# google/bayesnf

Hardware: AMD Instinct MI355X
Metric: train-steps/sec x ensemble_size (member-steps/s, whole job) (higher is better)
Workload: dtype bf16; 1 GPU; C2 chickenpox-like MAP: N=10232 rows, D=3, F=57, width=512, depth=2, NORMAL, full batch, lr=0.005; members_per_gpu=64, ensemble_size=64, parallelism=ensemble-shard x1 (no data-path collective)

## Files before the change

bayesnf_amd/csrc/bnf_api.hip:

```cpp
#include <hip/hip_runtime.h>
#include <cstring>
#include <rocprim/device/device_radix_sort.hpp>
#include <rocprim/device/device_segmented_radix_sort.hpp>

#include <dlfcn.h>

#include <atomic>
#include <cmath>
#include <cstdarg>
#include <cstdio>
#include <cstdlib>
#include <cstring>
#include <string>
#include <vector>

#include "../../include/bnf.h"
#include "bnf_gemm.h"
#include "bnf_kernels.h"
#include "bnf_panel.h"
#include "bnf_gemm8.h"

using namespace bnf;

static thread_local char g_err[512] = "";
// ... 74 lines not shown
  void* H0 = nullptr; void* H0t = nullptr;
  const float* ext_eps = nullptr;
  const uint32_t* vi_keys = nullptr; int64_t vi_key_rows = 0, vi_key_t0 = 0;
  const uint32_t* vi_draw_keys = nullptr; int64_t vi_draw_rows = 0;
  const int32_t* row_tab = nullptr; int64_t row_tab_epochs = 0, row_tab_e0 = 0;
  const uint32_t* row_keys = nullptr; int64_t row_keys_epochs = 0, row_keys_e0 = 0; int32_t row_key_rounds = 0;
  uint32_t* perm_bits[2] = {nullptr, nullptr}; int32_t* perm_val[2] = {nullptr, nullptr};
  unsigned* perm_seg = nullptr; void* perm_tmp = nullptr; size_t perm_tmp_bytes = 0;
  bool perm_ready = false;
  size_t owned_bytes = 0;
  int32_t* perm = nullptr; int64_t perm_epoch = -1;
  int32_t* leaf_off = nullptr; uint8_t* leaf_id = nullptr; int32_t n_leaves = 0;
  bool adam_clear_all = false;
  bool h0l = false;
  bool fold0 = false;
  void* A[BNF_MAX_LAYERS]; void* H[BNF_MAX_LAYERS]; void* Ht[BNF_MAX_LAYERS];
  void* dZ[BNF_MAX_LAYERS]; void* dZt[BNF_MAX_LAYERS];
  void* Kn[BNF_MAX_LAYERS]; void* Kt[BNF_MAX_LAYERS];
  int64_t pack_batch[BNF_MAX_LAYERS];
  float* dH0 = nullptr; float* out = nullptr; float* ybat = nullptr; float* loss_raw = nullptr;
  float* vacc = nullptr; float* dv = nullptr;
  bool vi_sample_pack = true, vi_keep_z = false;
  bool panel = false;
  void* Wf[BNF_MAX_LAYERS]; void* Wb[BNF_MAX_LAYERS];
  void* park[BNF_MAX_LAYERS];
    unsigned long long* prof_buf = nullptr;
  double prof_gap[16] = {0, 0, 0, 0, 0, 0, 0, 0, 0, 0, 0, 0, 0, 0, 0, 0};
  double prof_blocks = 0;
  int prof_threads = 0;
  bool recompute_a0 = false;
  bool fuse_last = false;
  int num_cus = 256;
  int tn_ring = 1;
  int skinny = 1;
  int big_tiles = 1;
  float* scal = nullptr;
  StepState* step_state = nullptr;
  hipGraphExec_t graph_exec = nullptr;
  int64_t graph_cols = 0;
  float* graph_losses = nullptr;
  int graph_mode = 0;
  float* qscratch = nullptr;
  float* dbg_a = nullptr; float* dbg_b = nullptr;
  uint8_t* is_matrix = nullptr;
  size_t ws_bytes = 0;
  int ablate = 0;
// ... 45 lines not shown
    h->dZ[l] = fo ? nullptr : take((size_t)Ev * Bp * W * es);
    h->dZt[l] = nullptr;
    const int64_t npad = (l == 0) ? Fp : W;
    h->pack_batch[l] = npad * W;
    h->Kn[l] = h->panel ? nullptr : take((size_t)Ev * npad * W * es);
    h->Kt[l] = h->panel ? nullptr : take((size_t)Ev * npad * W * es);
  }
  for (int l = 0; l < h->L; ++l) {
    const int64_t npad = (l == 0) ? Fp : W;
    h->Wf[l] = h->panel ? take((size_t)Ev * npad * W * es) : nullptr;
    h->Wb[l] = h->panel ? take((size_t)Ev * npad * W * es) : nullptr;
    h->park[l] = (h->panel && !fo && l >= 1 && l < h->L - 1) ? take((size_t)Ev * Bp * W * es) : nullptr;
    h->Wf8[l] = (h->c8 && l >= 1) ? (uint8_t*)take((size_t)Ev * W * W) : nullptr;
    h->Wb8[l] = (h->c8 && l >= 1) ? (uint8_t*)take((size_t)Ev * W * W) : nullptr;
  }
  h->dH0 = fo ? nullptr : (float*)take((size_t)Ev * Fp * Bp * 4);
  h->out = (float*)take((size_t)Ev * Bp * 4);
  h->vacc = (float*)take((size_t)Ev * Bp * 4);
  h->dv = fo ? nullptr : (float*)take((size_t)Ev * Bp * 4);
  h->ybat = fo ? nullptr : (float*)take((size_t)Ev * Bp * 4);
  h->loss_raw = (float*)take((size_t)Ev * 4);
  h->qscratch = (float*)take((size_t)(4 * 1024 + 16) * 4);
  h->scal = (float*)take((size_t)Ev * kScalStride * 4);
  h->step_state = (StepState*)take(sizeof(StepState));
  h->dbg_a = (float*)take(256);
  h->is_matrix = (uint8_t*)take((size_t)P);
  h->fbmeta = h->fbmeta_h.empty() ? nullptr : (int32_t*)take(h->fbmeta_h.size() * 4);
  if (h->cfg.mode == BNF_MODE_VI) {
    h->leaf_off = (int32_t*)take(260 * 4);
    h->leaf_id = (uint8_t*)take((size_t)P);
  }
  return off;
}

struct LaunchScope {
  bnf_handle* h;
  int kid;
  hipEvent_t t0 = nullptr, t1 = nullptr;
  bool on;
  hipStream_t st;
  LaunchScope(bnf_handle* h_, int kid_, hipStream_t st_ = nullptr, bool use_st = false)
      : h(h_), kid(kid_), on(((h_->prof >> kid_) & 1u) != 0), st(use_st ? st_ : h_->stream) {
    if (!on) return;
    auto get = [&]() {
      if (h->pool_used == h->event_pool.size()) {
        hipEvent_t ev;
// ... 565 lines not shown
    jb.off_kernel[l] = h->nd.off_kernel[l];
    jb.n_in[l] = (l == 0) ? h->F : h->W;
    jb.n_pad[l] = (l == 0) ? h->Fp : h->W;
    jb.tile0[l] = tiles;
    tiles += (jb.n_pad[l] / 64) * (h->W / 64);
    jb.wf[l] = h->Wf[l]; jb.wb[l] = h->Wb[l]; jb.batch[l] = h->pack_batch[l];
  }
  jb.tile0[h->L] = tiles;
  jb.fold0 = h->fold0 ? 1 : 0; jb.F0n = h->F; jb.off_bias0 = h->nd.off_bias[0]; jb.off_ls0 = h->nd.off_ls[0];
  for (int l = 0; l < h->L; ++l) { jb.wf8[l] = h->Wf8[l]; jb.wb8[l] = h->Wb8[l]; }
  jb.batch8 = (int64_t)h->W * h->W;
  *n_tiles = tiles;
  return jb;
}
template <typename T>
static void run_pack_fragments(bnf_handle* h, const float* theta, int nmem) {
  LaunchScope ls(h, KID_PACK);
  int tiles = 0;
  const PackJobs jb = pack_jobs(h, &tiles);
  hipLaunchKernelGGL((k_pack_layers<T>), dim3((unsigned)tiles * (unsigned)nmem), dim3(256), 0, h->stream,
                     theta, (int64_t)h->Pf, jb, h->nd, h->scal);
}

template <int WN, int RT, bool H0L, bool DEEP, int CH, int FP, bool F0, bool C8 = false>
static void launch_panel_f(bnf_handle* h, const PanelArgs& pa) {
  constexpr int kLds = panel_lds_bytes(WN, RT, H0L, CH, FP);
  static_assert(kLds <= 160 * 1024, "LDS per workgroup");
  static std::atomic<uint64_t> attr_done{0};
  allow_lds(h, &k_panel_fwd_bwd<WN, RT, H0L, DEEP, CH, FP, F0, C8>, kLds, &attr_done);
  PanelArgs pa2 = pa;
  pa2.ablate = h->ablate;
  const unsigned blocks = (unsigned)(pa.members * pa.panels);
  {
    EpiArgs tmp{};
    phase_prof_begin(h, KID_PANEL, blocks, &tmp);
    pa2.prof = tmp.prof;
  }
  {
    LaunchScope ls(h, KID_PANEL);
    hipLaunchKernelGGL((k_panel_fwd_bwd<WN, RT, H0L, DEEP, CH, FP, F0, C8>), dim3(blocks), dim3(512), kLds, h->stream, pa2);
  }
  phase_prof_end(h, KID_PANEL, blocks, 512);
}
template <int WN, int RT, bool H0L, bool DEEP, int CH, int FP>
static void launch_panel_d(bnf_handle* h, const PanelArgs& pa) {
  if constexpr (H0L) {
    if (h->fold0) {
      if (pa.c8) {
        launch_panel_f<WN, RT, H0L, DEEP, CH, FP, true, true>(h, pa);
        return;
      }
      launch_panel_f<WN, RT, H0L, DEEP, CH, FP, true>(h, pa);
      return;
    }
  }
  launch_panel_f<WN, RT, H0L, DEEP, CH, FP, false>(h, pa);
}

template <int WN, int RT, bool H0L, int CH = 1, int FP = 64>
static void launch_panel(bnf_handle* h, const PanelArgs& pa) {
  if (pa.n_layers == 2) launch_panel_d<WN, RT, H0L, false, CH, FP>(h, pa);
  else launch_panel_d<WN, RT, H0L, true, CH, FP>(h, pa);
}

static void run_panel(bnf_handle* h, const float* theta, int nmem, const RowSrc& rs, float c,
// ... 214 lines not shown
  } else {
    run_pack<T>(h, thf, E);
    run_forward<T>(h, thf, E, rs, h->X, h->stab, h->y, h->B, true);
    run_backward<T>(h, thf, E, rs, h->B, c, sink);
  }
  fold_grad(h, E);
  AdamArgs a{};
  a.theta = h->params; a.m = h->state; a.v = h->state + (int64_t)E * h->P; a.grad = h->grad;
  a.stride = h->P; a.P = h->P; a.off_shape = h->nd.off_shape;
  const int64_t t = h->adam_t + 1;
  a.lr = h->cfg.learning_rate;
  a.bc1 = (float)(1.0 - std::pow(0.9, (double)t));
  a.bc2 = (float)(1.0 - std::pow(0.999, (double)t));
  a.prior_weight = h->cfg.prior_weight;
  a.loss = sink.loss; a.loss_stride = sink.stride; a.loss_scale = sink.scale;
  a.apply = apply ? 1 : 0; a.loss_raw = sink.raw; a.st = sink.st;
  a.keep_lo = a.keep_hi = 0;
  if (!h->pad && !h->adam_clear_all && h->ablate == 0)
    for (int l = 1; l < h->L; ++l)
      if (wgrad_splitk(h, E, l) == 1 && a.keep_hi == 0) {
        a.keep_lo = (h->nd.off_kernel[l] + 3) / 4 * 4;
        a.keep_hi = (h->nd.off_kernel[l] + h->W * h->W) / 4 * 4;
      }
  {
    LaunchScope ls(h, KID_ADAM);
    hipLaunchKernelGGL(k_adam_map, dim3(cdiv(cdiv(h->P, 4), 256 * BNF_ADAM_QUADS), (unsigned)E), dim3(256), 0, h->stream, a);
  }
  if (apply) h->adam_t = t;
  return BNF_OK;
}

static ViSegs vi_segments_all(const bnf_handle* h) {
  ViSegs sg{};
  sg.n = 1; sg.lo[0] = 0; sg.hi[0] = h->P;
  return sg;
}
static ViSegs vi_segments_between_kernels(const bnf_handle* h) {
  ViSegs sg{};
  int32_t at = 0;
  for (int l = 0; l < h->L; ++l) {
    sg.lo[sg.n] = at; sg.hi[sg.n] = h->nd.off_kernel[l]; ++sg.n;
    at = h->nd.off_kernel[l] + ((l == 0) ? h->F : h->W) * h->W;
  }
  sg.lo[sg.n] = at; sg.hi[sg.n] = h->P; ++sg.n;
  return sg;
}
static dim3 vi_sample_grid(const ViSegs& sg, int members) {
  int32_t longest = 1;
  for (int i = 0; i < sg.n; ++i) longest = std::max(longest, sg.hi[i] - sg.lo[i]);
// ... 234 lines not shown
    int want = cfg->pipeline;
    if (const char* pf = getenv("BNF_PIPELINE")) want = atoi(pf);
    if (want != 0 && want != 1 && want != 3) {
      delete h;
      return fail(BNF_ERR_INVALID, "pipeline %d (0 auto, 1 layers, 3 panel)", want);
    }
    const bool can_panel = !cfg->forward_only && h->bf16 && h->L >= 2 && (h->W == 256 || h->W == 512 || h->W == 1024) && h->Fp <= 128;
    if (want == 3 && !can_panel) {
      delete h;
      return fail(BNF_ERR_INVALID, "panel pipeline needs a bf16 training handle with depth >= 2, width 256/512/1024 and <= 128 features");
    }
    h->panel = can_panel && (want == 3 || want == 0);
    if (h->q8 && !h->panel && !cfg->forward_only) {
      delete h;
      return fail(BNF_ERR_INVALID, "dtype fp8 (fp8 operand storage for the weight gradients) needs the row-panel pipeline: "
                  "depth >= 2, width 256 / 512 / 1024 after padding to 64, <= 128 padded features");
    }
    if (h->panel) h->Bp = align_up(h->B, 256);
    h->c8 = h->q8 && h->panel && !(getenv("BNF_FP8_CONTRACT") && atoi(getenv("BNF_FP8_CONTRACT")) == 0);
    const bool fl_ok = h->bf16 ? fused_last_supported<bf16_t>(h->W) : fused_last_supported<float>(h->W);
    h->fuse_last = !cfg->forward_only && !h->panel && want == 0 && fl_ok;
    h->recompute_a0 = !cfg->forward_only && !h->panel && want == 0 && h->L >= 2 && h->Fp <= 128;
  }
  h->h0l = panel_h0l(h);
  h->fold0 = h->h0l && h->F + 2 <= h->Fp && !(getenv("BNF_PANEL_FOLD0") && atoi(getenv("BNF_PANEL_FOLD0")) == 0);
  h->c8 = h->c8 && h->fold0;
  if (h->h0l &&
      !(getenv("BNF_PANEL_FEATBWD") && atoi(getenv("BNF_PANEL_FEATBWD")) == 0)) {
    int in_group = -1;
    for (int g = 0; g < cfg->n_groups; ++g)
      if (cfg->group_kind[g] == BNF_GROUP_INPUT) in_group = g;
    if (in_group >= 0) {
      std::vector<int32_t>& m = h->fbmeta_h;
      const int Fp = h->Fp;
      m.assign(Fp * 4 + BNF_MAX_GROUPS, 0);
      auto put = [&](int col, int kind, int g, int d1, int d2, int partner, int ucol, float coef) {
        m[4 * col] = kind | (g << 8) | (d1 << 16) | (d2 << 24);
        m[4 * col + 1] = partner | (ucol << 8);
        memcpy(&m[4 * col + 2], &coef, 4);
      };
      for (int c = 0; c < Fp; ++c) put(c, kFbNone, 0xff, 0xff, 0xff, 0, 0, 0.f);
      const int cin = cfg->group_col0[in_group];
      for (int g = 0; g < cfg->n_groups; ++g) {
        const int c0 = cfg->group_col0[g], nc = cfg->group_ncols[g];
        m[4 * Fp + g] = cfg->group_scale_off[g];
        switch (cfg->group_kind[g]) {
// ... 809 lines not shown
```

bayesnf_amd/csrc/bnf_kernels.h:

```cpp
#pragma once

#include "bnf_device.h"
#include "../../include/bnf.h"

namespace bnf {

constexpr int kScalGroup = BNF_MAX_LAYERS + 2;
constexpr int kScalInput = kScalGroup + BNF_MAX_GROUPS;
constexpr int kScalGfac = kScalInput + BNF_MAX_INPUTS;
constexpr int kScalStride = kScalGfac + BNF_MAX_GROUPS;

__device__ __forceinline__ void sincos_rev(float x, float* s, float* c) {
  sincosf(6.28318530717958647692f * x, s, c);
}

struct NetDev {
  int32_t D, F, Fp, W, Wt, depth, P, n_groups, n_freqs, n_interact, obs;
  int32_t group_kind[BNF_MAX_GROUPS], group_arg[BNF_MAX_GROUPS], group_ncols[BNF_MAX_GROUPS],
      group_col0[BNF_MAX_GROUPS], group_scale_off[BNF_MAX_GROUPS];
  int32_t fdeg[BNF_MAX_INPUTS];
  float in_scale[BNF_MAX_INPUTS];
  int32_t interact[BNF_MAX_INTERACT][2];
  int32_t off_lns, off_shape, off_infl;
  int32_t off_bias[BNF_MAX_LAYERS + 1], off_kernel[BNF_MAX_LAYERS + 1], off_ls[BNF_MAX_LAYERS];
// ... 553 lines not shown
  }
  theta_pad[(int64_t)e * Pp + j] = v;
}
__global__ void k_fold_grad(float* __restrict__ grad_pad, int64_t Pp, const int32_t* __restrict__ fold_src,
                            float* __restrict__ grad, int64_t P) {
  const int e = blockIdx.y;
  const int64_t i = (int64_t)blockIdx.x * blockDim.x + threadIdx.x;
  if (i >= P) return;
  grad[(int64_t)e * P + i] = grad_pad[(int64_t)e * Pp + fold_src[i]];
}

struct AdamArgs {
  float* theta; float* m; float* v; float* grad;
  int64_t stride;
  int32_t P;
  int32_t off_shape;
  float lr, bc1, bc2;
  float prior_weight;
  float* loss; int64_t loss_stride; float loss_scale;
  int32_t apply;
  float* loss_raw;
  const StepState* st;
  int32_t keep_lo, keep_hi;
};

__global__ void k_step_advance(StepState* st) {
  if (threadIdx.x == 0 && blockIdx.x == 0) {
    const long long t = st->t + 1;
    st->t = t;
    st->col += 1;
    st->bc1 = (float)(1.0 - pow(0.9, (double)t));
    st->bc2 = (float)(1.0 - pow(0.999, (double)t));
  }
}

#ifndef BNF_ADAM_QUADS
#define BNF_ADAM_QUADS 4
#endif
__global__ __launch_bounds__(256) void k_adam_map(AdamArgs a) {
  __shared__ float red[4];
  const int e = blockIdx.y;
  const float bc1 = a.st ? a.st->bc1 : a.bc1, bc2 = a.st ? a.st->bc2 : a.bc2;
  float lp = 0.f;
#pragma unroll
  for (int qd = 0; qd < BNF_ADAM_QUADS; ++qd) {
  const int p0 = ((blockIdx.x * BNF_ADAM_QUADS + qd) * blockDim.x + threadIdx.x) * 4;
  if (p0 < a.P) {
    const int nv = min(4, a.P - p0);
    const int64_t i0 = (int64_t)e * a.stride + p0;
    float th[4], g[4], m[4], v[4];
    load4u(a.theta + i0, nv, th); load4u(a.grad + i0, nv, g);
    if (a.apply) { load4u(a.m + i0, nv, m); load4u(a.v + i0, nv, v); }
    const float ibc1 = 1.0f / bc1, ibc2 = 1.0f / bc2;
#pragma unroll
    for (int k = 0; k < 4; ++k) {
      if (a.prior_weight != 0.f && k < nv) {
        const float z = th[k] - ((p0 + k) == a.off_shape ? -1.5f : 0.f);
        const float az = fabsf(z);
        const float e = __builtin_amdgcn_exp2f(-1.44269504088896340736f * az);
        const float r = __builtin_amdgcn_rcpf(1.0f + e);
        g[k] += a.prior_weight * copysignf((1.0f - e) * r, z);
        lp += -az - 1.38629436111989061883f * __builtin_amdgcn_logf(1.0f + e);
      }
      if (a.apply) {
        m[k] = 0.9f * m[k] + 0.1f * g[k];
        v[k] = 0.999f * v[k] + 0.001f * g[k] * g[k];
        th[k] = th[k] - a.lr * (m[k] * ibc1) * __builtin_amdgcn_rcpf(__builtin_amdgcn_sqrtf(v[k] * ibc2) + 1e-8f);
        g[k] = 0.f;
      }
    }
    if (!(a.apply && p0 >= a.keep_lo && p0 < a.keep_hi)) store4u(a.grad + i0, nv, g);
    if (a.apply) {
      store4u(a.theta + i0, nv, th);
      store4u<true>(a.m + i0, nv, m);
      store4u<true>(a.v + i0, nv, v);
    }
  }
  }
  const float s = wave_sum(lp);
  if ((threadIdx.x & 63) == 0) red[threadIdx.x >> 6] = s;
  __syncthreads();
  if (threadIdx.x == 0 && a.prior_weight != 0.f) {
    const float t = -(a.prior_weight) * (red[0] + red[1] + red[2] + red[3]);
    atomicAdd(&a.loss[(int64_t)e * a.loss_stride + (a.st ? a.st->col : 0)], a.loss_scale * t);
    if (a.loss_raw) atomicAdd(&a.loss_raw[e], t);
  }
}

__device__ __forceinline__ float hw_exp_neg_abs(float x) { return __builtin_amdgcn_exp2f(-1.44269504088896340736f * fabsf(x)); }
__device__ __forceinline__ float hw_log1p_of_exp(float t) { return 0.69314718055994530942f * __builtin_amdgcn_logf(1.0f + t); }
__device__ __forceinline__ float hw_softplus(float x) { return fmaxf(x, 0.f) + hw_log1p_of_exp(hw_exp_neg_abs(x)); }
__device__ __forceinline__ float hw_sigmoid(float x) {
  const float t = hw_exp_neg_abs(x), r = __builtin_amdgcn_rcpf(1.0f + t);
  return x >= 0.f ? r : t * r;
}
__device__ __forceinline__ float vi_sigma(float rho) { return 1e-4f + hw_softplus(rho); }

struct ViSegs {
  int32_t n;
  int32_t lo[BNF_MAX_LAYERS + 2], hi[BNF_MAX_LAYERS + 2];
};
__global__ __launch_bounds__(256) void k_vi_sample(const float* __restrict__ mu,
                                                   const float* __restrict__ rho, int32_t P,
                                                   int32_t S, uint64_t seed, int64_t member_offset,
                                                   uint64_t step, uint32_t stream,
                                                   float* __restrict__ z, int64_t z_member_stride,
// ... 511 lines not shown
```

bayesnf_amd/csrc/bnf_panel.h:

```cpp
#pragma once

#include <type_traits>

#include "bnf_gemm.h"
#include "bnf_kernels.h"

namespace bnf {

struct PanelArgs {
  int32_t F, Fp, B, panels, members;
  int32_t Wt;
  const float* theta;
  int64_t theta_stride;
  const float* scal;
  int32_t n_layers;
  int32_t off_bias[BNF_MAX_LAYERS], off_ls[BNF_MAX_LAYERS];
  int32_t off_bias_out, off_ko, off_os, off_law;
  int32_t off_lns, off_shape, off_infl, obs;
  const bf16_t* H0;
  const bf16_t* H0rm;
  int64_t h0_batch;
  const bf16_t* Wf[BNF_MAX_LAYERS];
  const bf16_t* Wb[BNF_MAX_LAYERS];
  int64_t w0_batch, w1_batch;
// ... 355 lines not shown
  step(1, std::false_type{}, std::integral_constant<int, 1>{});
#pragma unroll 1
  for (int ks = 2; ks < KS64; ks += 2) {
    step(ks, std::false_type{}, std::integral_constant<int, 0>{});
    step(ks + 1, std::false_type{}, std::integral_constant<int, 1>{});
  }
}

struct L0Blk {
  bf16x8 a[4], b[4];
};
__device__ __forceinline__ void l0_load(L0Blk& bk, const char* h0row, const char* w, int ks) {
#pragma unroll
  for (int u = 0; u < 4; ++u) {
    bk.a[u] = *reinterpret_cast<const bf16x8*>(h0row + (size_t)(ks + u) * 1024);
    bk.b[u] = *reinterpret_cast<const bf16x8*>(w + (size_t)(ks + u) * 1024);
  }
}
__device__ __forceinline__ void l0_mma(f32x16& a0, const L0Blk& bk) {
#pragma unroll
  for (int u = 0; u < 4; ++u) a0 = __builtin_amdgcn_mfma_f32_32x32x16_bf16(bk.a[u], bk.b[u], a0, 0, 0, 0);
}

template <int WN, int RT, bool H0L, bool DEEP = false, int CH = 1, int FP = 64, bool F0 = false, bool C8 = false>
__global__ __launch_bounds__(512, 2) void k_panel_fwd_bwd(const PanelArgs a) {
  static_assert(!F0 || H0L, "the folded layer 0 needs the LDS feature panel");
  constexpr int W = 64 * WN * CH, RB = 8 / WN, WR = 32 * RT, BM = WR * RB;
  constexpr int kSlabs = WN * CH;
  constexpr int kPitchE = W + 8;
  constexpr int kPitchB = kPitchE * 2;
  constexpr int kPitch8 = W + 16;
  constexpr int KS1 = W / 16;
  constexpr int kHalves = (RT + 1) / 2;
  extern __shared__ __attribute__((aligned(16))) char smem[];
#ifndef BNF_MARK0_AT
#define BNF_MARK0_AT 0
#endif
  if (BNF_MARK0_AT == 1) BNF_MARK(a, 0);
  bf16_t* tile = reinterpret_cast<bf16_t*>(smem);
  constexpr int kImageB = BM * kPitchB > 8 * 64 * kRowDotPitch * 4 ? BM * kPitchB : 8 * 64 * kRowDotPitch * 4;
  float* xs = reinterpret_cast<float*>(smem + kImageB);
  float* s_part = xs;
  float* s_dv = s_part + BM * kSlabs;
  float* s_col = s_dv + BM;
  float* s_sc = s_col + 2 * RB * W;
  constexpr int kH0Pitch = FP * 2 + 16;
  constexpr int KS0c = FP / 16;
// ... 756 lines not shown
#pragma unroll
    for (int i = 0; i < RT; ++i) {
      int tile_off = (rbase + i * 32 + 4 * kg) * kPitchE;
      asm volatile("" : "+v"(tile_off));
      bf16_t* tile_i = tile + tile_off;
#pragma unroll
      for (int rg = 0; rg < 4; ++rg) {
        const int lr = rbase + i * 32 + 8 * rg + 4 * kg;
        const f32x4 dv4 = *reinterpret_cast<const f32x4*>(s_dv + lr);
#pragma unroll
        for (int j = 0; j < 2; ++j) {
          const int lc = cbase + j * 32 + frow;
#pragma unroll
          for (int q = 0; q < 4; q += 2) {
            f32x2 tv = {acc[i][j][rg * 4 + q], acc[i][j][rg * 4 + q + 1]};
            asm volatile("" : "+v"(tv));
            const f32x2 dv2 = {dv4[q], dv4[q + 1]};
            const ActCore2 c = act_core2_pkclamp(tv);
            const f32x2 s = kLn2 * c.mxt + c.dl;
            const f32x2 dg = gkc[j] * (c.r - c.r * c.r) + gka[j] * c.dl;
            const f32x2 z = dv2 * dg;
            cr[j] += dv2 * c.r;
            cs[j] += dv2 * s;
            sg[j] += z * tv;
            cp[j] += z;
            if constexpr (C8) {
              store_pair_p8(lr + q, lc, z.x * inv_qdz, z.y * inv_qdz, std::true_type{});
            } else {
              store_pair_pk(tile_i + (8 * rg + q) * kPitchE + lc, tile_i + (8 * rg + q + 1) * kPitchE + lc, z.x, z.y);
            }
          }
        }
        asm volatile("" : "+v"(cr[0]), "+v"(cr[1]), "+v"(sg[0]), "+v"(sg[1]), "+v"(cp[0]), "+v"(cp[1]),
                     "+v"(cs[0]), "+v"(cs[1]));
        if (BNF_EPI_FENCE_EVERY == 1 || (rg & 1)) __builtin_amdgcn_sched_barrier(0);
        if (rg == 1 && i > 0) block_to_global(L, a.dZ[LL], i - 1, cbase);
      }
    }
    block_to_global(L, a.dZ[LL], RT - 1, cbase);
    if (hc == CH - 1 && !c8) ring_prefetch(wbl(LL), lane);
    const float crj[2] = {cr[0].x + cr[0].y, cr[1].x + cr[1].y}, csj[2] = {cs[0].x + cs[0].y, cs[1].x + cs[1].y};
    float wsa = kvn[0] * (2.f * crj[0] + csj[0]) + kvn[1] * (2.f * crj[1] + csj[1]);
    float wsg = (kLn2 / gamma1) * ((sg[0].x + sg[0].y) + (sg[1].x + sg[1].y));
    float dv_rows = 0.f;
#pragma unroll
    for (int w2 = 0; w2 < (WR + 63) / 64; ++w2) dv_rows += s_sc[(rbase / 64 + w2) * 5 + 2];
#pragma unroll
    for (int j = 0; j < 2; ++j) {
      float b = cp[j].x + cp[j].y, k = ak.c1 * crj[j] + ak.alpha * csj[j];
      b += __shfl_xor(b, 32, 64);
      k += __shfl_xor(k, 32, 64);
      k += ak.c0 * dv_rows;
      if (lane < 32) {
        s_col[rb * W + cbase + j * 32 + lane] = b;
        s_col[(RB + rb) * W + cbase + j * 32 + lane] = k;
      }
    }
    wsa_all += wave_sum_dpp(wsa);
    wsg_all += wave_sum_dpp(wsg);
    if (hc == CH - 1 && lane == 0) {
      s_sc[32 + wave * 2] = wsa_all;
      s_sc[33 + wave * 2] = wsg_all;
    }
  }
  }
  if constexpr (C8 && kL1T) {
    lds_barrier();
    const LaneCtx L = lane_ctx();
    const int frow = L.frow, kg = L.kg;
#pragma unroll
    for (int i = 0; i < RT; ++i) {
      const float dvs = s_dv[rbase + i * 32 + frow] * inv_qdz;
      char* rowp8 = smem + (rbase + i * 32 + frow) * kPitch8 + slab(0) * 64 + 4 * kg;
#pragma unroll
      for (int j = 0; j < 2; ++j)
#pragma unroll
        for (int rg = 0; rg < 4; ++rg) {
          const f32x2 z0 = f32x2{accs[0][i][j][rg * 4], accs[0][i][j][rg * 4 + 1]} * dvs;
          const f32x2 z1 = f32x2{accs[0][i][j][rg * 4 + 2], accs[0][i][j][rg * 4 + 3]} * dvs;
          int pk = __builtin_amdgcn_cvt_pk_bf8_f32(z0.x, z0.y, 0, false);
          pk = __builtin_amdgcn_cvt_pk_bf8_f32(z1.x, z1.y, pk, true);
          *reinterpret_cast<int*>(rowp8 + j * 32 + 8 * rg) = pk;
        }
    }
  }
  BNF_MARK(a, 8);
  lds_barrier();
  for (int c = tid; !kL1T && c < W; c += 512) {
    float b = 0.f, k = 0.f;
#pragma unroll
    for (int r = 0; r < RB; ++r) {
      b += s_col[r * W + c];
      k += s_col[(RB + r) * W + c];
    }
    atomicAdd(&gr[a.off_bias[LL] + c], b);
    atomicAdd(&gr[a.off_ko + c], k * inv_sw);
  }
  float ta1 = 0.f;
  if (tid == 0) {
    float tg = 0.f;
#pragma unroll
    for (int w2 = 0; w2 < 8; ++w2) {
      ta1 += s_sc[32 + w2 * 2];
      tg += s_sc[33 + w2 * 2];
    }
    float ko_all = 0.f;
#pragma unroll
    for (int w2 = 0; w2 < WN; ++w2) ko_all += s_sc[48 + w2];
    ta1 -= 2.f * inv_sw * ko_all * dv_all;
    atomicAdd(&gr[a.off_ls[LL]], dgam1 * tg);
  }

#pragma unroll 1
  for (int l = LL - 1; DEEP && l >= 1; --l) {
    if constexpr (c8) contract_all8(a.Wb8[l + 1] + (int64_t)e * a.w8_batch, std::false_type{}, std::true_type{});
    else contract_all(wbl(l + 1));
    const LaneCtx L = lane_ctx();
    const int lane = L.lane, frow = L.frow, kg = L.kg;
    u32x4 pv[2][2];
    auto park_load = [&](const bf16_t* pk, int t2, u32x4 (&dst)[2]) {
      const u32x4* src = reinterpret_cast<const u32x4*>(pk + (min(t2, 2 * RT - 1) * 2 * 64 + lane) * 8);
      dst[0] = __builtin_nontemporal_load(src);
      dst[1] = __builtin_nontemporal_load(src + 64);
    };
    park_load(park_ptr(l, 0), 0, pv[0]);
    if (kL1T && l == LL - 1) copy_panel_by_early_waves(a.dZ[LL]);
    lds_barrier();
    float sa_all = 0.f, sg_all = 0.f;
#pragma unroll
    for (int hc = 0; hc < CH; ++hc) {
      const int cbase = slab(hc) * 64;
      f32x16 (&acc)[RT][2] = accs[hc];
      const bf16_t* pk = park_ptr(l, hc);
// ... 6 lines not shown
        int tile_off = (rbase + i * 32 + 4 * kg) * kPitchE;
        asm volatile("" : "+v"(tile_off));
        bf16_t* tile_i = tile + tile_off;
#pragma unroll
        for (int j = 0; j < 2; ++j) {
          const int t2 = 2 * i + j;
          park_load(pk, t2 + 1, pv[(t2 + 1) & 1]);
          const u32x4 (&cur)[2] = pv[t2 & 1];
          const int lc = cbase + j * 32 + frow;
#pragma unroll
          for (int rg = 0; rg < 4; ++rg) {
            const int lr = rbase + i * 32 + 8 * rg + 4 * kg;
#pragma unroll
            for (int q = 0; q < 4; q += 2) {
              const uint32_t w = cur[rg >> 1][(rg & 1) * 2 + (q >> 1)];
              const f32x2 tv = {__builtin_bit_cast(float, w << 16), __builtin_bit_cast(float, w & 0xffff0000u)};
              const f32x2 raw = {acc[i][j][rg * 4 + q], acc[i][j][rg * 4 + q + 1]};
              const ActCore2 c = act_core2_pkclamp(tv);
              const f32x2 s = kLn2 * c.mxt + c.dl;
              const f32x2 dg = gzc * (c.r - c.r * c.r) + gza * c.dl;
              const f32x2 z = raw * dg;
              sa2 += raw * (2.f * c.r + s);
              sacc += raw;
              sg2 += z * tv;
              cs2[j] += z;
              if constexpr (C8) store_pair_p8(lr + q, lc, z.x * inv_qdz, z.y * inv_qdz, std::true_type{});
              else store_pair_pk(tile_i + (8 * rg + q) * kPitchE + lc, tile_i + (8 * rg + q + 1) * kPitchE + lc, z.x, z.y);
            }
            asm volatile("" : "+v"(sa2), "+v"(sg2), "+v"(sacc), "+v"(cs2[0]), "+v"(cs2[1]));
            __builtin_amdgcn_sched_barrier(0);
          }
          if (j == 0 && i > 0) block_to_global(L, a.dZ[l], i - 1, cbase);
        }
      }
      block_to_global(L, a.dZ[l], RT - 1, cbase);
      if (hc == CH - 1 && !c8) ring_prefetch(wbl(l), lane);
#pragma unroll
      for (int j = 0; j < 2; ++j) {
        float c = cs2[j].x + cs2[j].y;
        c += __shfl_xor(c, 32, 64);
        if (lane < 32) s_col[rb * W + cbase + j * 32 + lane] = c;
      }
      sa_all += wave_sum_dpp(inv_sw * ((sa2.x + sa2.y) - 2.f * (sacc.x + sacc.y)));
      sg_all += wave_sum_dpp((kLn2 / gl) * (sg2.x + sg2.y));
      if (hc == CH - 1 && lane == 0) {
        s_sc[32 + wave * 2] = sa_all;
        s_sc[33 + wave * 2] = sg_all;
      }
    }
    lds_barrier();
    for (int c = tid; c < W; c += 512) {
      float b = 0.f;
#pragma unroll
      for (int r = 0; r < RB; ++r) b += s_col[r * W + c];
      atomicAdd(&gr[a.off_bias[l] + c], b);
    }
    if (tid == 0) {
      float tg = 0.f;
#pragma unroll
      for (int w2 = 0; w2 < 8; ++w2) {
        ta1 += s_sc[32 + w2 * 2];
        tg += s_sc[33 + w2 * 2];
      }
      atomicAdd(&gr[a.off_ls[l]], sigmoidf(th[a.off_ls[l]]) / sc[l] * tg);
    }
  }

  BNF_MARK(a, 9);
  if constexpr (c8)
    contract_all8(a.Wb8[1] + (int64_t)e * a.w8_batch, std::integral_constant<bool, F0>{}, std::true_type{});
  else
    contract_all_t(wbl(1), std::integral_constant<bool, F0>{});
  BNF_MARK(a, 10);
  const LaneCtx L2 = lane_ctx(0);
  l0_weights(L2);
  if (kL1T && LL == 1) copy_panel_by_early_waves(a.dZ[1]);
  lds_barrier();

  float sa0_all = 0.f, sg0_all = 0.f;
#pragma unroll
  for (int hc = 0; hc < CH; ++hc) {
    const int cbase = slab(hc) * 64;
    f32x16 (&acc)[RT][2] = accs[hc];
    const LaneCtx L = (hc == 0) ? L2 : lane_ctx(hc);
    if (hc > 0) l0_weights(L);
    const int lane = L.lane, frow = L.frow, kg = L.kg;
    const float gs0 = gamma0 * inv_sf * kLog2e;
// ... 19 lines not shown
          else {
#pragma unroll
            for (int r = 0; r < 16; ++r) a0[r] = 0.25f;
          }
        }
        if constexpr (F0) {
          bf16_t* rowp = tile + (rbase + i * 32 + frow) * kPitchE + cbase + j * 32 + 4 * kg;
#pragma unroll
          for (int rg = 0; rg < 4; ++rg) {
            f32x2 zq[2];
#pragma unroll
            for (int q = 0; q < 4; q += 2) {
              const f32x2 raw = {acc[i][j][rg * 4 + q], acc[i][j][rg * 4 + q + 1]};
              const f32x2 tv = {a0[rg * 4 + q], a0[rg * 4 + q + 1]};
              f32x2 z = raw;
              if (!BNF_ABL(a, 2)) {
                const ActCore2 c = act_core2_pkclamp(tv);
                const f32x2 s = kLn2 * c.mxt + c.dl;
                const f32x2 dg = gzc * (c.r - c.r * c.r) + gza * c.dl;
                z = raw * dg;
                sa2 += raw * (2.f * c.r + s);
              }
              sacc += raw;
              sg2 += z * tv;
              zq[q >> 1] = z;
            }
            if (!BNF_ABL(a, 4)) store_quad_pk(rowp + 8 * rg, zq[0].x, zq[0].y, zq[1].x, zq[1].y);
            asm volatile("" : "+v"(sa2), "+v"(sg2), "+v"(sacc));
            if (BNF_EPI_FENCE_EVERY == 1 || (rg & 1)) __builtin_amdgcn_sched_barrier(0);
          }
          if (j == 0 && i > 0) block_to_global(L, a.dZ[0], i - 1, cbase);
          continue;
        }
        const int lc = cbase + j * 32 + frow;
#pragma unroll
        for (int rg = 0; rg < 4; ++rg) {
          const int lr = rbase + i * 32 + 8 * rg + 4 * kg;
#pragma unroll
          for (int q = 0; q < 4; q += 2) {
            const f32x2 raw = {acc[i][j][rg * 4 + q], acc[i][j][rg * 4 + q + 1]};
            const f32x2 tv = f32x2{a0[rg * 4 + q], a0[rg * 4 + q + 1]} * gs0 + gb0[j];
            f32x2 z = raw;
            if (!BNF_ABL(a, 2)) {
              const ActCore2 c = act_core2_pkclamp(tv);
              const f32x2 s = kLn2 * c.mxt + c.dl;
              const f32x2 dg = gzc * (c.r - c.r * c.r) + gza * c.dl;
              z = raw * dg;
              sa2 += raw * (2.f * c.r + s);
            }
            sacc += raw;
            sg2 += z * tv;
            cs2[j] += z;
            if (!BNF_ABL(a, 4)) store_pair_pk(tile + (lr + q) * kPitchE + lc, tile + (lr + q + 1) * kPitchE + lc, z.x, z.y);
          }
          asm volatile("" : "+v"(sa2), "+v"(sg2), "+v"(sacc), "+v"(cs2[0]), "+v"(cs2[1]));
          if (BNF_EPI_FENCE_EVERY == 1 || (rg & 1)) __builtin_amdgcn_sched_barrier(0);
        }
        if (j == 0 && i > 0) block_to_global(L, a.dZ[0], i - 1, cbase);
      }
    }
    block_to_global(L, a.dZ[0], RT - 1, cbase);
    BNF_MARK(a, 11);
    if constexpr (!F0) {
#pragma unroll
      for (int j = 0; j < 2; ++j) {
        float c = cs2[j].x + cs2[j].y;
        c += __shfl_xor(c, 32, 64);
        if (lane < 32) s_col[rb * W + cbase + j * 32 + lane] = c;
      }
    }
    sa0_all += wave_sum_dpp(inv_sw * ((sa2.x + sa2.y) - 2.f * (sacc.x + sacc.y)));
    sg0_all += wave_sum_dpp((kLn2 / gamma0) * (sg2.x + sg2.y));
    if (hc == CH - 1 && lane == 0) {
      s_sc[32 + wave * 2] = sa0_all;
      s_sc[33 + wave * 2] = sg0_all;
    }
  }
  int4 md_red = {0, 0, 0, 0};
  {
    const LaneCtx L = lane_ctx();
    const int lane = L.lane, frow = L.frow, kg = L.kg;
    const int ct = a.Fp / 32;
    const int n_t = (BM / 32) * ct;
    float* dh0 = a.dH0t + (int64_t)e * a.dh0_batch;
    constexpr int KC = KS1 < 32 ? KS1 : 32;
    bf16x8 fb[KC];
    const PanelW wb0w = panel_wbase(wb0);
    auto load_b = [&](int t, int k0) {
      const uint32_t o = (uint32_t)((t % ct) * KS1 + k0) * 1024u;
#pragma unroll
      for (int u = 0; u < KC; ++u) fb[u] = panel_wload(wb0w, o + (uint32_t)u * 1024u, (uint32_t)lane * 16u);
    };
    load_b(wave, 0);
    int4 md_first = {0, 0, 0, 0};
    if constexpr (H0L) {
      if (a.fbmeta) {
        md_first = *reinterpret_cast<const int4*>(a.fbmeta + 4 * ((wave % ct) * 32 + frow));
        if (wave < FP / 64) md_red = *reinterpret_cast<const int4*>(a.fbmeta + 4 * (wave * 64 + lane));
      }
    }
    BNF_MARK(a, 12);
    lds_barrier();
    if constexpr (!F0) {
      for (int c = tid; c < W; c += 512) {
        float b = 0.f;
#pragma unroll
        for (int r = 0; r < RB; ++r) b += s_col[r * W + c];
        atomicAdd(&gr[a.off_bias[0] + c], b);
      }
    }
    if (tid == 0) {
      float ta = ta1, tg = 0.f;
#pragma unroll
      for (int w2 = 0; w2 < 8; ++w2) {
        ta += s_sc[32 + w2 * 2];
        tg += s_sc[33 + w2 * 2];
      }
      atomicAdd(&gr[a.off_law], alpha * (1.f - alpha) * ta);
      atomicAdd(&gr[a.off_ls[0]], dgam0 * tg);
    }
    for (int t = wave; t < n_t; t += 8) {
      const int mi = t / ct, ni = t - mi * ct;
      const char* ap = smem + (mi * 32 + frow) * kPitchB + kg * 16;
      f32x16 c0, c1;
#pragma unroll
      for (int r = 0; r < 16; ++r) c0[r] = c1[r] = 0.f;
#pragma unroll
      for (int k0 = 0; k0 < KS1; k0 += KC) {
        if (t != wave || k0 != 0) load_b(t, k0);
#pragma unroll
        for (int u = 0; u < KC; u += 2) {
          const bf16x8 fa0 = *reinterpret_cast<const bf16x8*>(ap + (k0 + u) * 32);
          const bf16x8 fa1 = *reinterpret_cast<const bf16x8*>(ap + (k0 + u + 1) * 32);
          c0 = __builtin_amdgcn_mfma_f32_32x32x16_bf16(fa0, fb[u], c0, 0, 0, 0);
          c1 = __builtin_amdgcn_mfma_f32_32x32x16_bf16(fa1, fb[u + 1], c1, 0, 0, 0);
        }
      }
      if constexpr (H0L) {
        if (a.fbmeta) {
          const int f = ni * 32 + frow;
          const int4 md = (t == wave) ? md_first : *reinterpret_cast<const int4*>(a.fbmeta + 4 * f);
          const char* hc = h0s + (mi * 32 + 4 * kg) * kH0Pitch;
// ... 71 lines not shown
```

Baseline: 36410 member-steps/s.

## Derive layer-scale gradients from grad·theta dot products in Adam instead of panel epilogue

Removes the per-element z*tv accumulation, its wave reductions and atomics for the layer-scale gradient from the fused panel forward/backward kernel. The Adam kernel instead accumulates per-layer dot products of kernel/bias gradients with parameters, and a small per-member kernel reconstructs each layer-scale gradient as sigmoid/softplus times that dot and applies Adam to it. This lightens the hot epilogue but adds range checks and extra reductions/atomics in Adam, one more launch per step, and relies on an algebraic identity that must hold for the scaling parameterization.

```diff
diff --git a/bayesnf_amd/csrc/bnf_api.hip b/bayesnf_amd/csrc/bnf_api.hip
--- a/bayesnf_amd/csrc/bnf_api.hip
+++ b/bayesnf_amd/csrc/bnf_api.hip
@@ -120,6 +120,8 @@
   float* vacc = nullptr; float* dv = nullptr;
   bool vi_sample_pack = true, vi_keep_z = false;
   bool panel = false;
+  bool scale_dots = false;
+  float* sdot = nullptr;
   void* Wf[BNF_MAX_LAYERS]; void* Wb[BNF_MAX_LAYERS];
   void* park[BNF_MAX_LAYERS];
     unsigned long long* prof_buf = nullptr;
@@ -211,6 +213,7 @@
   h->loss_raw = (float*)take((size_t)Ev * 4);
   h->qscratch = (float*)take((size_t)(4 * 1024 + 16) * 4);
   h->scal = (float*)take((size_t)Ev * kScalStride * 4);
+  h->sdot = h->scale_dots ? (float*)take((size_t)Ev * BNF_MAX_LAYERS * 4) : nullptr;
   h->step_state = (StepState*)take(sizeof(StepState));
   h->dbg_a = (float*)take(256);
   h->is_matrix = (uint8_t*)take((size_t)P);
@@ -822,12 +825,12 @@
                      theta, (int64_t)h->Pf, jb, h->nd, h->scal);
 }
 
-template <int WN, int RT, bool H0L, bool DEEP, int CH, int FP, bool F0, bool C8 = false>
-static void launch_panel_f(bnf_handle* h, const PanelArgs& pa) {
+template <int WN, int RT, bool H0L, bool DEEP, int CH, int FP, bool F0, bool C8 = false, bool GS = true>
+static void launch_panel_g(bnf_handle* h, const PanelArgs& pa) {
   constexpr int kLds = panel_lds_bytes(WN, RT, H0L, CH, FP);
   static_assert(kLds <= 160 * 1024, "LDS per workgroup");
   static std::atomic<uint64_t> attr_done{0};
-  allow_lds(h, &k_panel_fwd_bwd<WN, RT, H0L, DEEP, CH, FP, F0, C8>, kLds, &attr_done);
+  allow_lds(h, &k_panel_fwd_bwd<WN, RT, H0L, DEEP, CH, FP, F0, C8, GS>, kLds, &attr_done);
   PanelArgs pa2 = pa;
   pa2.ablate = h->ablate;
   const unsigned blocks = (unsigned)(pa.members * pa.panels);
@@ -838,9 +841,19 @@
   }
   {
     LaunchScope ls(h, KID_PANEL);
-    hipLaunchKernelGGL((k_panel_fwd_bwd<WN, RT, H0L, DEEP, CH, FP, F0, C8>), dim3(blocks), dim3(512), kLds, h->stream, pa2);
+    hipLaunchKernelGGL((k_panel_fwd_bwd<WN, RT, H0L, DEEP, CH, FP, F0, C8, GS>), dim3(blocks), dim3(512), kLds, h->stream, pa2);
   }
   phase_prof_end(h, KID_PANEL, blocks, 512);
+}
+template <int WN, int RT, bool H0L, bool DEEP, int CH, int FP, bool F0, bool C8 = false>
+static void launch_panel_f(bnf_handle* h, const PanelArgs& pa) {
+  if constexpr (!C8) {
+    if (h->scale_dots) {
+      launch_panel_g<WN, RT, H0L, DEEP, CH, FP, F0, C8, false>(h, pa);
+      return;
+    }
+  }
+  launch_panel_g<WN, RT, H0L, DEEP, CH, FP, F0, C8, true>(h, pa);
 }
 template <int WN, int RT, bool H0L, bool DEEP, int CH, int FP>
 static void launch_panel_d(bnf_handle* h, const PanelArgs& pa) {
@@ -1101,9 +1114,20 @@
         a.keep_lo = (h->nd.off_kernel[l] + 3) / 4 * 4;
         a.keep_hi = (h->nd.off_kernel[l] + h->W * h->W) / 4 * 4;
       }
+  if (h->scale_dots) {
+    a.dots = h->sdot; a.n_layers = h->L; a.db_n = h->Wt;
+    a.ls_lo = a.ls_hi = h->cfg.off_layer_scale[0];
+    for (int l = 0; l < h->L; ++l) {
+      a.dk_lo[l] = h->cfg.off_kernel[l]; a.dk_n[l] = ((l == 0) ? h->F : h->Wt) * h->Wt;
+      a.db_lo[l] = h->cfg.off_bias[l];
+      a.off_ls[l] = h->cfg.off_layer_scale[l];
+      a.ls_lo = std::min(a.ls_lo, a.off_ls[l]); a.ls_hi = std::max(a.ls_hi, a.off_ls[l]);
+    }
+  }
   {
     LaunchScope ls(h, KID_ADAM);
     hipLaunchKernelGGL(k_adam_map, dim3(cdiv(cdiv(h->P, 4), 256 * BNF_ADAM_QUADS), (unsigned)E), dim3(256), 0, h->stream, a);
+    if (h->scale_dots) hipLaunchKernelGGL(k_scale_adam, dim3((unsigned)E), dim3(64), 0, h->stream, a);
   }
   if (apply) h->adam_t = t;
   return BNF_OK;
@@ -1384,6 +1408,7 @@
     h->fuse_last = !cfg->forward_only && !h->panel && want == 0 && fl_ok;
     h->recompute_a0 = !cfg->forward_only && !h->panel && want == 0 && h->L >= 2 && h->Fp <= 128;
   }
+  h->scale_dots = h->panel && cfg->mode == BNF_MODE_MAP && !h->q8;
   h->h0l = panel_h0l(h);
   h->fold0 = h->h0l && h->F + 2 <= h->Fp && !(getenv("BNF_PANEL_FOLD0") && atoi(getenv("BNF_PANEL_FOLD0")) == 0);
   h->c8 = h->c8 && h->fold0;
diff --git a/bayesnf_amd/csrc/bnf_kernels.h b/bayesnf_amd/csrc/bnf_kernels.h
--- a/bayesnf_amd/csrc/bnf_kernels.h
+++ b/bayesnf_amd/csrc/bnf_kernels.h
@@ -599,6 +599,12 @@
   float* loss_raw;
   const StepState* st;
   int32_t keep_lo, keep_hi;
+  float* dots;
+  int32_t n_layers;
+  int32_t dk_lo[BNF_MAX_LAYERS], dk_n[BNF_MAX_LAYERS];
+  int32_t db_lo[BNF_MAX_LAYERS], db_n;
+  int32_t off_ls[BNF_MAX_LAYERS];
+  int32_t ls_lo, ls_hi;
 };
 
 __global__ void k_step_advance(StepState* st) {
@@ -619,18 +625,52 @@
   const int e = blockIdx.y;
   const float bc1 = a.st ? a.st->bc1 : a.bc1, bc2 = a.st ? a.st->bc2 : a.bc2;
   float lp = 0.f;
+  float dot[BNF_MAX_LAYERS];
+#pragma unroll
+  for (int l = 0; l < BNF_MAX_LAYERS; ++l) dot[l] = 0.f;
+  uint32_t dot_hit = 0;
 #pragma unroll
   for (int qd = 0; qd < BNF_ADAM_QUADS; ++qd) {
-  const int p0 = ((blockIdx.x * BNF_ADAM_QUADS + qd) * blockDim.x + threadIdx.x) * 4;
+  const int q_lo = (blockIdx.x * BNF_ADAM_QUADS + qd) * blockDim.x * 4, q_hi = q_lo + blockDim.x * 4;
+  const int p0 = q_lo + threadIdx.x * 4;
+  uint32_t hit = 0;
+  if (a.dots) {
+#pragma unroll
+    for (int l = 0; l < BNF_MAX_LAYERS; ++l)
+      if (l < a.n_layers && ((q_lo < a.dk_lo[l] + a.dk_n[l] && q_hi > a.dk_lo[l]) ||
+                             (q_lo < a.db_lo[l] + a.db_n && q_hi > a.db_lo[l]))) hit |= 1u << l;
+  }
+  dot_hit |= hit;
   if (p0 < a.P) {
     const int nv = min(4, a.P - p0);
     const int64_t i0 = (int64_t)e * a.stride + p0;
     float th[4], g[4], m[4], v[4];
     load4u(a.theta + i0, nv, th); load4u(a.grad + i0, nv, g);
     if (a.apply) { load4u(a.m + i0, nv, m); load4u(a.v + i0, nv, v); }
+    uint32_t skip = 0;
+    if (a.dots) {
+#pragma unroll
+      for (int l = 0; l < BNF_MAX_LAYERS; ++l) {
+        if ((hit >> l) & 1) {
+#pragma unroll
+          for (int k = 0; k < 4; ++k) {
+            const bool in = (uint32_t)(p0 + k - a.dk_lo[l]) < (uint32_t)a.dk_n[l] ||
+                            (uint32_t)(p0 + k - a.db_lo[l]) < (uint32_t)a.db_n;
+            dot[l] += (in && k < nv) ? g[k] * th[k] : 0.f;
+          }
+        }
+      }
+      if (p0 + 3 >= a.ls_lo && p0 <= a.ls_hi) {
+        for (int l = 0; l < a.n_layers; ++l) {
+          const int k = a.off_ls[l] - p0;
+          if (k >= 0 && k < 4) skip |= 1u << k;
+        }
+      }
+    }
     const float ibc1 = 1.0f / bc1, ibc2 = 1.0f / bc2;
 #pragma unroll
     for (int k = 0; k < 4; ++k) {
+      if ((skip >> k) & 1) continue;
       if (a.prior_weight != 0.f && k < nv) {
         const float z = th[k] - ((p0 + k) == a.off_shape ? -1.5f : 0.f);
         const float az = fabsf(z);
@@ -659,6 +699,52 @@
   __syncthreads();
   if (threadIdx.x == 0 && a.prior_weight != 0.f) {
     const float t = -(a.prior_weight) * (red[0] + red[1] + red[2] + red[3]);
+    atomicAdd(&a.loss[(int64_t)e * a.loss_stride + (a.st ? a.st->col : 0)], a.loss_scale * t);
+    if (a.loss_raw) atomicAdd(&a.loss_raw[e], t);
+  }
+  if (dot_hit) {
+#pragma unroll
+    for (int l = 0; l < BNF_MAX_LAYERS; ++l) {
+      if ((dot_hit >> l) & 1) {
+        const float d = wave_sum(dot[l]);
+        __syncthreads();
+        if ((threadIdx.x & 63) == 0) red[threadIdx.x >> 6] = d;
+        __syncthreads();
+        if (threadIdx.x == 0) atomicAdd(&a.dots[e * BNF_MAX_LAYERS + l], (red[0] + red[1]) + (red[2] + red[3]));
+      }
+    }
+  }
+}
+
+__global__ __launch_bounds__(64) void k_scale_adam(AdamArgs a) {
+  const int e = blockIdx.x, l = threadIdx.x;
+  const float bc1 = a.st ? a.st->bc1 : a.bc1, bc2 = a.st ? a.st->bc2 : a.bc2;
+  float lp = 0.f;
+  if (l < a.n_layers) {
+    const int64_t i = (int64_t)e * a.stride + a.off_ls[l];
+    float th = a.theta[i];
+    float* dp = a.dots + e * BNF_MAX_LAYERS + l;
+    float g = a.grad[i] + sigmoidf(th) / softplusf(th) * *dp;
+    *dp = 0.f;
+    if (a.prior_weight != 0.f) {
+      const float az = fabsf(th);
+      const float ex = __builtin_amdgcn_exp2f(-1.44269504088896340736f * az);
+      const float r = __builtin_amdgcn_rcpf(1.0f + ex);
+      g += a.prior_weight * copysignf((1.0f - ex) * r, th);
+      lp = -az - 1.38629436111989061883f * __builtin_amdgcn_logf(1.0f + ex);
+    }
+    if (a.apply) {
+      const float m = 0.9f * a.m[i] + 0.1f * g;
+      const float v = 0.999f * a.v[i] + 0.001f * g * g;
+      th = th - a.lr * (m * (1.0f / bc1)) * __builtin_amdgcn_rcpf(__builtin_amdgcn_sqrtf(v * (1.0f / bc2)) + 1e-8f);
+      a.theta[i] = th; a.m[i] = m; a.v[i] = v;
+      g = 0.f;
+    }
+    a.grad[i] = g;
+  }
+  const float s = wave_sum(lp);
+  if (threadIdx.x == 0 && a.prior_weight != 0.f) {
+    const float t = -(a.prior_weight) * s;
     atomicAdd(&a.loss[(int64_t)e * a.loss_stride + (a.st ? a.st->col : 0)], a.loss_scale * t);
     if (a.loss_raw) atomicAdd(&a.loss_raw[e], t);
   }
diff --git a/bayesnf_amd/csrc/bnf_panel.h b/bayesnf_amd/csrc/bnf_panel.h
--- a/bayesnf_amd/csrc/bnf_panel.h
+++ b/bayesnf_amd/csrc/bnf_panel.h
@@ -401,7 +401,7 @@
   for (int u = 0; u < 4; ++u) a0 = __builtin_amdgcn_mfma_f32_32x32x16_bf16(bk.a[u], bk.b[u], a0, 0, 0, 0);
 }
 
-template <int WN, int RT, bool H0L, bool DEEP = false, int CH = 1, int FP = 64, bool F0 = false, bool C8 = false>
+template <int WN, int RT, bool H0L, bool DEEP = false, int CH = 1, int FP = 64, bool F0 = false, bool C8 = false, bool GS = true>
 __global__ __launch_bounds__(512, 2) void k_panel_fwd_bwd(const PanelArgs a) {
   static_assert(!F0 || H0L, "the folded layer 0 needs the LDS feature panel");
   constexpr int W = 64 * WN * CH, RB = 8 / WN, WR = 32 * RT, BM = WR * RB;
@@ -1204,7 +1204,7 @@
             const f32x2 z = dv2 * dg;
             cr[j] += dv2 * c.r;
             cs[j] += dv2 * s;
-            sg[j] += z * tv;
+            if constexpr (GS) sg[j] += z * tv;
             cp[j] += z;
             if constexpr (C8) {
               store_pair_p8(lr + q, lc, z.x * inv_qdz, z.y * inv_qdz, std::true_type{});
@@ -1213,8 +1213,11 @@
             }
           }
         }
-        asm volatile("" : "+v"(cr[0]), "+v"(cr[1]), "+v"(sg[0]), "+v"(sg[1]), "+v"(cp[0]), "+v"(cp[1]),
-                     "+v"(cs[0]), "+v"(cs[1]));
+        if constexpr (GS)
+          asm volatile("" : "+v"(cr[0]), "+v"(cr[1]), "+v"(sg[0]), "+v"(sg[1]), "+v"(cp[0]), "+v"(cp[1]),
+                       "+v"(cs[0]), "+v"(cs[1]));
+        else
+          asm volatile("" : "+v"(cr[0]), "+v"(cr[1]), "+v"(cp[0]), "+v"(cp[1]), "+v"(cs[0]), "+v"(cs[1]));
         if (BNF_EPI_FENCE_EVERY == 1 || (rg & 1)) __builtin_amdgcn_sched_barrier(0);
         if (rg == 1 && i > 0) block_to_global(L, a.dZ[LL], i - 1, cbase);
       }
@@ -1239,10 +1242,10 @@
       }
     }
     wsa_all += wave_sum_dpp(wsa);
-    wsg_all += wave_sum_dpp(wsg);
+    if constexpr (GS) wsg_all += wave_sum_dpp(wsg);
     if (hc == CH - 1 && lane == 0) {
       s_sc[32 + wave * 2] = wsa_all;
-      s_sc[33 + wave * 2] = wsg_all;
+      if constexpr (GS) s_sc[33 + wave * 2] = wsg_all;
     }
   }
   }
@@ -1284,13 +1287,13 @@
 #pragma unroll
     for (int w2 = 0; w2 < 8; ++w2) {
       ta1 += s_sc[32 + w2 * 2];
-      tg += s_sc[33 + w2 * 2];
+      if constexpr (GS) tg += s_sc[33 + w2 * 2];
     }
     float ko_all = 0.f;
 #pragma unroll
     for (int w2 = 0; w2 < WN; ++w2) ko_all += s_sc[48 + w2];
     ta1 -= 2.f * inv_sw * ko_all * dv_all;
-    atomicAdd(&gr[a.off_ls[LL]], dgam1 * tg);
+    if constexpr (GS) atomicAdd(&gr[a.off_ls[LL]], dgam1 * tg);
   }
 
 #pragma unroll 1
@@ -1343,12 +1346,13 @@
               const f32x2 z = raw * dg;
               sa2 += raw * (2.f * c.r + s);
               sacc += raw;
-              sg2 += z * tv;
+              if constexpr (GS) sg2 += z * tv;
               cs2[j] += z;
               if constexpr (C8) store_pair_p8(lr + q, lc, z.x * inv_qdz, z.y * inv_qdz, std::true_type{});
               else store_pair_pk(tile_i + (8 * rg + q) * kPitchE + lc, tile_i + (8 * rg + q + 1) * kPitchE + lc, z.x, z.y);
             }
-            asm volatile("" : "+v"(sa2), "+v"(sg2), "+v"(sacc), "+v"(cs2[0]), "+v"(cs2[1]));
+            if constexpr (GS) asm volatile("" : "+v"(sa2), "+v"(sg2), "+v"(sacc), "+v"(cs2[0]), "+v"(cs2[1]));
+            else asm volatile("" : "+v"(sa2), "+v"(sacc), "+v"(cs2[0]), "+v"(cs2[1]));
             __builtin_amdgcn_sched_barrier(0);
           }
           if (j == 0 && i > 0) block_to_global(L, a.dZ[l], i - 1, cbase);
@@ -1363,10 +1367,10 @@
         if (lane < 32) s_col[rb * W + cbase + j * 32 + lane] = c;
       }
       sa_all += wave_sum_dpp(inv_sw * ((sa2.x + sa2.y) - 2.f * (sacc.x + sacc.y)));
-      sg_all += wave_sum_dpp((kLn2 / gl) * (sg2.x + sg2.y));
+      if constexpr (GS) sg_all += wave_sum_dpp((kLn2 / gl) * (sg2.x + sg2.y));
       if (hc == CH - 1 && lane == 0) {
         s_sc[32 + wave * 2] = sa_all;
-        s_sc[33 + wave * 2] = sg_all;
+        if constexpr (GS) s_sc[33 + wave * 2] = sg_all;
       }
     }
     lds_barrier();
@@ -1381,9 +1385,9 @@
 #pragma unroll
       for (int w2 = 0; w2 < 8; ++w2) {
         ta1 += s_sc[32 + w2 * 2];
-        tg += s_sc[33 + w2 * 2];
-      }
-      atomicAdd(&gr[a.off_ls[l]], sigmoidf(th[a.off_ls[l]]) / sc[l] * tg);
+        if constexpr (GS) tg += s_sc[33 + w2 * 2];
+      }
+      if constexpr (GS) atomicAdd(&gr[a.off_ls[l]], sigmoidf(th[a.off_ls[l]]) / sc[l] * tg);
     }
   }
 
@@ -1449,11 +1453,12 @@
                 sa2 += raw * (2.f * c.r + s);
               }
               sacc += raw;
-              sg2 += z * tv;
+              if constexpr (GS) sg2 += z * tv;
               zq[q >> 1] = z;
             }
             if (!BNF_ABL(a, 4)) store_quad_pk(rowp + 8 * rg, zq[0].x, zq[0].y, zq[1].x, zq[1].y);
-            asm volatile("" : "+v"(sa2), "+v"(sg2), "+v"(sacc));
+            if constexpr (GS) asm volatile("" : "+v"(sa2), "+v"(sg2), "+v"(sacc));
+            else asm volatile("" : "+v"(sa2), "+v"(sacc));
             if (BNF_EPI_FENCE_EVERY == 1 || (rg & 1)) __builtin_amdgcn_sched_barrier(0);
           }
           if (j == 0 && i > 0) block_to_global(L, a.dZ[0], i - 1, cbase);
@@ -1476,11 +1481,12 @@
               sa2 += raw * (2.f * c.r + s);
             }
             sacc += raw;
-            sg2 += z * tv;
+            if constexpr (GS) sg2 += z * tv;
             cs2[j] += z;
             if (!BNF_ABL(a, 4)) store_pair_pk(tile + (lr + q) * kPitchE + lc, tile + (lr + q + 1) * kPitchE + lc, z.x, z.y);
           }
-          asm volatile("" : "+v"(sa2), "+v"(sg2), "+v"(sacc), "+v"(cs2[0]), "+v"(cs2[1]));
+          if constexpr (GS) asm volatile("" : "+v"(sa2), "+v"(sg2), "+v"(sacc), "+v"(cs2[0]), "+v"(cs2[1]));
+          else asm volatile("" : "+v"(sa2), "+v"(sacc), "+v"(cs2[0]), "+v"(cs2[1]));
           if (BNF_EPI_FENCE_EVERY == 1 || (rg & 1)) __builtin_amdgcn_sched_barrier(0);
         }
         if (j == 0 && i > 0) block_to_global(L, a.dZ[0], i - 1, cbase);
@@ -1497,10 +1503,10 @@
       }
     }
     sa0_all += wave_sum_dpp(inv_sw * ((sa2.x + sa2.y) - 2.f * (sacc.x + sacc.y)));
-    sg0_all += wave_sum_dpp((kLn2 / gamma0) * (sg2.x + sg2.y));
+    if constexpr (GS) sg0_all += wave_sum_dpp((kLn2 / gamma0) * (sg2.x + sg2.y));
     if (hc == CH - 1 && lane == 0) {
       s_sc[32 + wave * 2] = sa0_all;
-      s_sc[33 + wave * 2] = sg0_all;
+      if constexpr (GS) s_sc[33 + wave * 2] = sg0_all;
     }
   }
   int4 md_red = {0, 0, 0, 0};
@@ -1541,10 +1547,10 @@
 #pragma unroll
       for (int w2 = 0; w2 < 8; ++w2) {
         ta += s_sc[32 + w2 * 2];
-        tg += s_sc[33 + w2 * 2];
+        if constexpr (GS) tg += s_sc[33 + w2 * 2];
       }
       atomicAdd(&gr[a.off_law], alpha * (1.f - alpha) * ta);
-      atomicAdd(&gr[a.off_ls[0]], dgam0 * tg);
+      if constexpr (GS) atomicAdd(&gr[a.off_ls[0]], dgam0 * tg);
     }
     for (int t = wave; t < n_t; t += 8) {
       const int mi = t / ct, ni = t - mi * ct;
```

Result: no change. 36440 member-steps/s (median of 2 runs) (+0.1%).
